# Innoptech/OpenFDCM

Hardware: AMD Instinct MI355X
Metric: template matches/sec (DT3 build + DefaultMatch/BatchOptimize search per frame) (higher is better)
Workload: dtype f32

## Files before the change

### openfdcm_amd/csrc/fdcm_capi.cpp

```cpp
#include <algorithm>
#include <cfloat>
#include <cmath>
#include <cstdlib>
#include <condition_variable>
#include <cstring>
#include <deque>
#include <functional>
#include <mutex>
#include <numeric>
#include <thread>

#include "fdcm_internal.h"
#include "fdcm_sweep.h"

namespace fdcm {
int device_cus(int device) {
    static std::mutex mu;
    static int cached[64] = {};
    std::lock_guard<std::mutex> lock(mu);
    int& c = cached[device & 63];
    if (c <= 0) FDCM_HIP(hipDeviceGetAttribute(&c, hipDeviceAttributeMultiprocessorCount, device));
    return c;
}
const char* last_error_cstr();
static thread_local int g_device = 0;

template <class F>
static int guarded(F&& f) {
    try {
        f();
        return FDCM_OK;
    } catch (const HipError& e) {
        set_error(std::string("HIP error: ") + hipGetErrorString(e.code) + " in " + e.what);
        return FDCM_EHIP;
    } catch (const std::string& s) {
        set_error(s);
        return FDCM_EINVAL;
    } catch (const std::exception& e) {
        set_error(e.what());
        return FDCM_EINTERNAL;
    } catch (...) {
        set_error("unknown error");
        return FDCM_EINTERNAL;
    }
}

static void require(bool ok, const char* msg) {
    if (!ok) throw std::string(msg);
}

template <class F>
static void records_call(fdcm_match** out, F&& call) {
    *out = nullptr;
    try {
        call();
    } catch (...) {
        result_release(*out);
        *out = nullptr;
        throw;
    }
    if (!*out) *out = result_acquire(sizeof(fdcm_match));
}

static void upload_keys_only(fdcm_featuremap* fm) {
    BuildPlan keys_only;
    keys_only.W = fm->W; keys_only.H = fm->H; keys_only.m = fm->m; keys_only.keys = fm->keys;
    const BuildLayout L = build_layout(keys_only, fm->distance, 3);
    fm->off_keys = L.off_keys;
    fm->build.plan.reserve(std::max<size_t>(16, L.plan));
    if (!fm->keys.empty())
        FDCM_HIP(hipMemcpy((char*)fm->build.plan.p + fm->off_keys, fm->keys.data(), fm->keys.size() * sizeof(float), hipMemcpyHostToDevice));
}

static void destroy(fdcm_featuremap* fm) {
    if (!fm) return;
    (void)hipSetDevice(fm->device);
    if (fm->stream) (void)hipStreamSynchronize(fm->stream);
    if (fm->prep_stream) (void)hipStreamSynchronize(fm->prep_stream);
    fm->vol.release(); fm->ivol.release(); fm->build.release(); fm->search.release();
    fm->coverage.release(); fm->coverage_stage.release();
    if (fm->timing.created)
        for (auto& e : fm->timing.ev) (void)hipEventDestroy(e);
    if (fm->stream) (void)hipStreamDestroy(fm->stream);
// ... 339 lines not shown
}

int fdcm_featuremap_from_slices(const float* keys, int64_t depth, const float* volume_host, int64_t width,
                                int64_t height, const float scene_translation[2], fdcm_featuremap** out) {
    fdcm_featuremap* fm = nullptr;
    int rc = guarded([&] {
        require(out && scene_translation, "null argument");
        require(depth >= 0 && width >= 0 && height >= 0, "negative size");
        require(depth == 0 || (keys && volume_host), "null keys/volume");
        for (int64_t i = 1; i < depth; ++i) require(keys[i - 1] < keys[i], "keys must be strictly ascending (std::map order)");
        fm = new fdcm_featuremap();
        fm->device = g_device;
        FDCM_HIP(hipSetDevice(fm->device));
        fm->depth_param = depth; fm->m = depth; fm->W = width; fm->H = height;
        fm->tx = scene_translation[0]; fm->ty = scene_translation[1];
        fm->keys.assign(keys, keys + depth);
        require(width <= 16384 && height <= 16384, "feature size above 16384 is not supported");
        const size_t sl = ivol_slice_floats(width, height);
        if (depth && sl) {
            fm->vol.reserve((size_t)depth * sl * sizeof(float));
            std::vector<float> tmp(sl, 0.f);
            for (int64_t k = 0; k < depth; ++k) {
                slice_from_xy(volume_host + (size_t)k * width * height, tmp.data(), width, height);
                FDCM_HIP(hipMemcpy(fm->vol.as<float>() + (size_t)k * sl, tmp.data(), sl * sizeof(float), hipMemcpyHostToDevice));
            }
        }
        fm->holds = VolStage::integrated;
        upload_keys_only(fm);
        *out = fm;
    });
    if (rc != FDCM_OK) { destroy(fm); if (out) *out = nullptr; }
    return rc;
}

static void check_offsets(const int64_t* off, int64_t n, const char* what) {
    require(off != nullptr, what);
    require(off[0] == 0, "offsets[0] must be 0");
    for (int64_t i = 0; i < n; ++i) require(off[i] <= off[i + 1], "offsets must be ascending");
}

int fdcm_featuremap_minmax_translation_batch(const fdcm_featuremap* fm, const float* tmpl_lines, const int64_t* line_offsets,
                                             int64_t n_templates, const float* align_vecs, float* out_minmax) {
    return guarded([&] {
        require(fm != nullptr, "featuremap is null");
        require(n_templates >= 0, "negative template count");
        if (n_templates == 0) return;
        check_offsets(line_offsets, n_templates, "line_offsets is null");
        require(line_offsets[n_templates] == 0 || tmpl_lines, "tmpl_lines is null");
        require(align_vecs && out_minmax, "null align_vecs/out_minmax");
        run_minmax(const_cast<fdcm_featuremap*>(fm), tmpl_lines, line_offsets, n_templates, align_vecs, out_minmax);
    });
}

int fdcm_featuremap_minmax_translation(const fdcm_featuremap* fm, const float* tmpl_lines, int64_t n_lines,
                                       const float align_vec[2], float out_minmax[2]) {
    const int64_t off[2] = {0, n_lines};
    if (n_lines < 0) { set_error("negative line count"); return FDCM_EINVAL; }
    return fdcm_featuremap_minmax_translation_batch(fm, tmpl_lines, off, 1, align_vec, out_minmax);
}

int fdcm_featuremap_evaluate(const fdcm_featuremap* fm, const float* tmpl_lines, const int64_t* line_offsets,
                             int64_t n_templates, const float* translations, const int64_t* translation_offsets,
                             float* scores_out) {
    return guarded([&] {
        require(fm != nullptr, "featuremap is null");
        require(n_templates >= 0, "negative template count");
        if (n_templates == 0) return;
        check_offsets(line_offsets, n_templates, "line_offsets is null");
        check_offsets(translation_offsets, n_templates, "translation_offsets is null");
        require(line_offsets[n_templates] == 0 || tmpl_lines, "tmpl_lines is null");
        require(translation_offsets[n_templates] == 0 || (translations && scores_out), "null translations/scores_out");
        run_evaluate(const_cast<fdcm_featuremap*>(fm), tmpl_lines, line_offsets, n_templates, translations, translation_offsets,
                     scores_out);
    });
}

static int create_templates(const float* lines, const int64_t* offsets, int64_t n_templates, const float* caps, fdcm_templates** out,
                            int32_t footprint = FDCM_FOOTPRINT_BOX) {
    fdcm_templates* t = nullptr;
    int rc = guarded([&] {
        require(out != nullptr, "out is null");
        require(n_templates >= 0 && (n_templates == 0 || offsets), "bad offsets");
        t = new fdcm_templates();
        t->device = g_device;
        t->footprint = footprint;
        FDCM_HIP(hipSetDevice(t->device));
        t->T = n_templates;
        t->offsets.assign(n_templates + 1, 0);
        for (int64_t i = 0; i <= n_templates && offsets; ++i) t->offsets[i] = offsets[i];
        require(t->offsets[0] == 0, "offsets[0] must be 0");
        for (int64_t i = 0; i < n_templates; ++i) require(t->offsets[i] <= t->offsets[i + 1], "offsets must be ascending");
        t->n_lines = t->offsets[n_templates];
        require(t->n_lines == 0 || lines, "lines is null");
        t->lines.assign(lines, lines + 4 * t->n_lines);
        t->lengths.resize((size_t)t->n_lines);
        t->sorted.resize((size_t)t->n_lines);
        for (int64_t i = 0; i < t->n_lines; ++i) {
            const float dx = lines[4 * i + 2] - lines[4 * i], dy = lines[4 * i + 3] - lines[4 * i + 1];
            t->lengths[i] = std::sqrt(dx * dx + dy * dy);
        }
        t->caps.assign((size_t)t->n_lines, f_inf());
        for (int64_t i = 0; i < t->n_lines && caps; ++i) {
            t->caps[i] = caps[i] == 0.f ? 0.f : caps[i];
            t->capped = t->capped || caps[i] < f_inf();
        }
        std::vector<long> ind;
        for (int64_t i = 0; i < n_templates; ++i) {
            const int64_t l0 = t->offsets[i], n = t->offsets[i + 1] - l0;
            t->max_lines = std::max(t->max_lines, n);
            ind.resize((size_t)n);
            std::iota(ind.begin(), ind.end(), 0);
            const float* len = t->lengths.data() + l0;
            std::sort(ind.begin(), ind.end(), [len](long const i1, long const i2) { return len[i1] > len[i2]; });
            for (int64_t j = 0; j < n; ++j) t->sorted[l0 + j] = (int32_t)ind[j];
        }
        t->d_lines.reserve(std::max<size_t>(16, t->lines.size() * 4));
        t->d_offsets.reserve((size_t)(n_templates + 1) * 8);
        t->d_lengths.reserve(std::max<size_t>(16, t->lengths.size() * 4));
        t->d_sorted.reserve(std::max<size_t>(16, t->sorted.size() * 4));
        if (t->n_lines) {
            FDCM_HIP(hipMemcpy(t->d_lines.p, t->lines.data(), t->lines.size() * 4, hipMemcpyHostToDevice));
            FDCM_HIP(hipMemcpy(t->d_lengths.p, t->lengths.data(), t->lengths.size() * 4, hipMemcpyHostToDevice));
            FDCM_HIP(hipMemcpy(t->d_sorted.p, t->sorted.data(), t->sorted.size() * 4, hipMemcpyHostToDevice));
        }
        FDCM_HIP(hipMemcpy(t->d_offsets.p, t->offsets.data(), (size_t)(n_templates + 1) * 8, hipMemcpyHostToDevice));
        *out = t;
    });
    if (rc != FDCM_OK) { if (t) fdcm_templates_free(t); if (out) *out = nullptr; }
    return rc;
}

int fdcm_templates_create(const float* lines, const int64_t* offsets, int64_t n_templates, fdcm_templates** out) {
    return create_templates(lines, offsets, n_templates, nullptr, out);
}

int fdcm_templates_create_capped(const float* lines, const int64_t* offsets, int64_t n_templates, const float* caps,
                                 fdcm_templates** out) {
    int rc = guarded([&] {
        require(out != nullptr, "out is null");
        require(n_templates >= 0 && (n_templates == 0 || offsets), "bad offsets");
        if (!caps || n_templates == 0) return;
        require(offsets[0] == 0, "offsets[0] must be 0");
        for (int64_t i = 0; i < n_templates; ++i) require(offsets[i] <= offsets[i + 1], "offsets must be ascending");
        for (int64_t i = 0; i < offsets[n_templates]; ++i) require(caps[i] >= 0.f, "caps must be >= 0 or +inf, never NaN");
    });
    if (rc != FDCM_OK) { if (out) *out = nullptr; return rc; }
    return create_templates(lines, offsets, n_templates, caps, out);
}

int fdcm_templates_create_shaped(const float* lines, const int64_t* offsets, int64_t n_templates, const float* caps, int32_t footprint,
                                 fdcm_templates** out) {
    int rc = guarded([&] {
        require(footprint == FDCM_FOOTPRINT_BOX || footprint == FDCM_FOOTPRINT_HULL, "footprint must be FDCM_FOOTPRINT_BOX or FDCM_FOOTPRINT_HULL");
        require(out != nullptr, "out is null");
        require(n_templates >= 0 && (n_templates == 0 || offsets), "bad offsets");
        if (!caps || n_templates == 0) return;
        require(offsets[0] == 0, "offsets[0] must be 0");
        for (int64_t i = 0; i < n_templates; ++i) require(offsets[i] <= offsets[i + 1], "offsets must be ascending");
        for (int64_t i = 0; i < offsets[n_templates]; ++i) require(caps[i] >= 0.f, "caps must be >= 0 or +inf, never NaN");
    });
    if (rc != FDCM_OK) { if (out) *out = nullptr; return rc; }
    return create_templates(lines, offsets, n_templates, caps, out, footprint);
}

int fdcm_templates_footprint_kind(const fdcm_templates* t, int32_t* kind) {
    return guarded([&] {
// ... 1235 lines not shown
```

### openfdcm_amd/csrc/fdcm_internal.h

```cpp
#pragma once
#include <hip/hip_runtime.h>
#include <stdint.h>
#include <algorithm>
#include <cstdlib>
#include <cstring>
#include <mutex>
#include <string>
#include <vector>

#include "../../include/fdcm.h"
#include "fdcm_math.h"

namespace fdcm {

void set_error(const std::string& msg);
struct HipError { hipError_t code; const char* what; int line; };
#define FDCM_HIP(call)                                                              \
    do {                                                                            \
        hipError_t e__ = (call);                                                    \
        if (e__ != hipSuccess) throw ::fdcm::HipError{e__, #call, __LINE__};        \
    } while (0)

struct TestSwitches {
    bool literal_sweep, sweep_order;
// ... 71 lines not shown
    std::vector<PropStep> prop;
    std::vector<IntegralDesc> integral;
    std::vector<LineBox> boxes;
    SeedSource seeds;
};

struct BuildLayout {
    bool empty = true;
    bool balanced = false;
    int HW64 = 0, slots = 0;
    long nchunks = 0;
    size_t vol = 0, ivol = 0, bitmap = 0, coldesc = 0, colmask = 0, offtab = 0, stack = 0;
    size_t labels = 0;
    size_t edge_parent = 0, edge_roots = 0;
    size_t pyr = 0, pyr_b = 0;
    size_t o_ent = 0, o_own = 0, o_ord = 0, o_cost = 0, o_steals = 0;
    size_t off_raster = 0, off_prop = 0, off_integral = 0, off_keys = 0, off_slice = 0, off_pixels = 0, off_cost = 0, plan = 0;
};
void make_build_plan(const float* lines, int64_t n, int64_t depth, float coeff, float padding, BuildPlan& plan);
void plan_keys(int64_t depth, std::vector<float>& keys);
void make_shape_plan(int64_t depth, float coeff, int64_t W, int64_t H, BuildPlan& plan);
void sweep_cost_proxy(const BuildPlan& plan, std::vector<int32_t>& cost);

FDCM_HD float lin_spaced_value(int mode, float low, float high, float step, int n, int i) {
    if (mode == 0) return low;
    const int size1 = (n == 1) ? 1 : n - 1;
    if (mode == 2) return (i == 0) ? low : (high - (float)(size1 - i) * step);
    return (i == size1) ? high : (low + (float)i * step);
}

static constexpr size_t kSlicePad = 1088;
FDCM_HD size_t ivol_slice_floats(int64_t W, int64_t H) { return (size_t)((W + 3) / 4) * (size_t)H * 4 + kSlicePad; }
FDCM_HD size_t ivol_index(int x, int y, int64_t H) { return ((size_t)(x >> 2) * (size_t)H + (size_t)y) * 4 + (size_t)(x & 3); }
inline void slice_to_xy(const float* il, float* xy, int64_t W, int64_t H) {
    for (int64_t x = 0; x < W; ++x)
        for (int64_t y = 0; y < H; ++y) xy[(size_t)x * H + y] = il[ivol_index((int)x, (int)y, H)];
}
inline void slice_from_xy(const float* xy, float* il, int64_t W, int64_t H) {
    for (int64_t x = 0; x < W; ++x)
        for (int64_t y = 0; y < H; ++y) il[ivol_index((int)x, (int)y, H)] = xy[(size_t)x * H + y];
}
enum class VolStage { none, transforms, propagated, integrated };

struct Timing { hipEvent_t ev[9] = {}; bool created = false; };

struct SweepHistory { long cost_chunks = 0; int cost_w = 0; size_t steals_off = 0; void reset() { *this = SweepHistory{}; } };
struct GroupTable { int m = 0, steps = 0; void reset() { *this = GroupTable{}; } };
struct BuildRecord {
    bool pending = false;
    bool seeds_fused = false;
    bool stage_events = false, total_events = false;
    float host_ms = 0.f;
    void reset() { *this = BuildRecord{}; }
};
struct BuildBuffers {
    DevBuf bitmap;
    DevBuf coldesc;
    DevBuf colmask;
    DevBuf labels;
    DevBuf edge_parent, edge_roots;
    DevBuf pyr;
    DevBuf offtab;
    DevBuf stack;
    DevBuf plan; PinnedBuf stage;
    void release() { for (DevBuf* b : {&bitmap, &coldesc, &colmask, &labels, &edge_parent, &edge_roots, &pyr, &offtab, &stack, &plan}) b->release(); stage.release(); }
};
struct SearchBuffers {
    DevBuf scene;
    DevBuf pairs;
    DevBuf records, flags;
    DevBuf out;
    DevBuf work;
    DevBuf tail, tail_out;
    DevBuf eval;
    DevBuf counter;
    DevBuf bins;
    DevBuf eval_spans;
    PinnedBuf stage, bins_stage, eval_stage;
    PinnedBuf cnt;
    void release() {
        for (DevBuf* b : {&scene, &pairs, &records, &flags, &out, &work, &tail, &tail_out, &eval, &eval_spans, &counter, &bins}) b->release();
        for (PinnedBuf* b : {&stage, &bins_stage, &eval_stage, &cnt}) b->release();
    }
};

}

struct fdcm_featuremap {
    int device = 0;
    hipStream_t stream = nullptr;
    hipStream_t prep_stream = nullptr;
    hipEvent_t prep_done = nullptr;
    int64_t depth_param = 0;
    float coeff = 0, padding = 0;
    int distance = 0;
    bool pixel_seeded = false;
    int want_stage_events = 1;
    bool shares_gpu = false;
    int64_t W = 0, H = 0, m = 0;
    float tx = 0, ty = 0;
    std::vector<float> keys;
    size_t off_keys = 0;
    fdcm::DevBuf vol;
    fdcm::DevBuf ivol;
    fdcm::VolStage holds = fdcm::VolStage::none;
    const float* current() const { return holds == fdcm::VolStage::propagated ? ivol.as<float>() : vol.as<float>(); }
    fdcm::BuildBuffers build;
    fdcm::SweepHistory sweep;
    fdcm::GroupTable groups;
    fdcm::BuildRecord built;
    int* steal_counter() const { return sweep.steals_off ? (int*)((char*)build.stack.p + sweep.steals_off) : nullptr; }
    fdcm::SearchBuffers search;
    fdcm::DevBuf coverage;
    fdcm::PinnedBuf coverage_stage;
    std::mutex seam_mutex;
    int64_t last_n_out = 0;
    fdcm::Timing timing;
    fdcm_build_timing last_build = {};
    fdcm_search_timing last_search = {};
};

struct fdcm_templates {
    int device = 0;
    int64_t T = 0, n_lines = 0, max_lines = 0;
    std::vector<float> lines;
    std::vector<int64_t> offsets;
    std::vector<float> lengths;
    std::vector<float> caps;
    bool capped = false;
    int32_t footprint = 0;
    std::vector<int32_t> sorted;
    fdcm::DevBuf d_lines, d_offsets, d_lengths, d_sorted;
};

namespace fdcm {
void ensure_stream(fdcm_featuremap* fm);
BuildLayout build_layout(const BuildPlan& plan, int distance, int stop_after);
void reserve_build(fdcm_featuremap* fm, const BuildLayout& L);
void run_build(fdcm_featuremap* fm, const BuildPlan& plan, int stop_after);
void launch_edge_labels(hipStream_t st, const uint8_t* image, int width, int height, int row_stride, const float* keys, int m,
                        const fdcm_edge_params& e, uint8_t* labels, int32_t* parent, uint32_t* roots);
void pyramid_size(int64_t width, int64_t height, int level, int64_t* w_out, int64_t* h_out);
const uint8_t* launch_pyramid(hipStream_t st, const uint8_t* image, int width, int height, int row_stride, int level, uint8_t* a, uint8_t* b,
                              uint8_t* last = nullptr);
void image_pyramid_host(int device, const uint8_t* image, int width, int height, int row_stride, bool on_device, int level, uint8_t* out,
                        bool out_on_device);
void launch_coldesc_labels(hipStream_t st, const uint8_t* labels, int width, int height, int border, void* desc, int W, int H,
                           int HW64, int m, unsigned* colmask, int* cost);
struct PixelScratch {
    DevBuf pixels, labels, keys, parent, counts, comps, out;
    ~PixelScratch();
    void take(DevBuf& b, size_t bytes, int id);
    const uint8_t* upload(const uint8_t* host_or_device, int width, int height, int& row_stride, bool on_device, const std::vector<float>* host_keys);
};
void edge_labels_host(int device, const uint8_t* image, int width, int height, int row_stride, int64_t depth, const fdcm_edge_params& e,
                      bool hysteresis, uint8_t* labels_out);
void lines_from_labels_host(int device, const uint8_t* labels, int width, int height, bool on_device, int m, const fdcm_line_params& lp,
                            float** lines, int64_t* n_lines);
void lines_from_image_host(int device, const uint8_t* image, int width, int height, int row_stride, bool on_device, int64_t depth,
                           const fdcm_edge_params& e, const fdcm_line_params& lp, float** lines, int64_t* n_lines);
void lines_last_timing(fdcm_lines_timing* out);
void finish_build(fdcm_featuremap* fm);
void sweep_order_counts(int64_t* from_history, int64_t* from_proxy);
int64_t search_capacity(const fdcm_templates* t, int64_t n_scene, int64_t maxT, int64_t maxS);
void run_search(fdcm_featuremap* fm, const fdcm_templates* t, const float* scene, int64_t n_scene, int64_t maxT,
                int64_t maxS, int optimizer, int64_t batch, int32_t base, fdcm_match* out_device, fdcm_match** out_host,
                int64_t* n_out);
void reserve_search(fdcm_featuremap* fm, const fdcm_templates* t, int64_t n_scene, int64_t maxT, int64_t maxS);
bool orientation_bins_on_host();
void reserve_eval(fdcm_featuremap* fm, size_t device_bytes, size_t stage_bytes);
void run_minmax(fdcm_featuremap* fm, const float* lines, const int64_t* offsets, int64_t T, const float* align, float* out);
void run_evaluate(fdcm_featuremap* fm, const float* lines, const int64_t* offsets, int64_t T, const float* translations,
                  const int64_t* tr_offsets, float* scores);
void exhaustive_window(fdcm_featuremap* fm, const fdcm_templates* t, int32_t sx, int32_t sy, fdcm_grid* out);
void run_score_map(fdcm_featuremap* fm, const fdcm_templates* t, const fdcm_rotations* rot, const fdcm_grid& g, float* out_host,
                   float* out_device);
void run_search_exhaustive(fdcm_featuremap* fm, const fdcm_templates* t, const fdcm_grid& g, int k, int32_t base,
                           fdcm_match** out, int64_t* n_out);
void run_search_exhaustive_peaks(fdcm_featuremap* fm, const fdcm_templates* t, const fdcm_grid& g, int k, int rx, int ry,
                                 int32_t base, fdcm_match** out, int64_t* n_out);
void exhaustive_rotations_window(fdcm_featuremap* fm, const fdcm_templates* t, const fdcm_rotations& rot, int32_t sx, int32_t sy,
                                 fdcm_grid* out);
void run_search_exhaustive_rotations(fdcm_featuremap* fm, const fdcm_templates* t, const fdcm_rotations& rot, const fdcm_grid& g,
                                     int k, int rx, int ry, int ra, int wrap, int32_t base, fdcm_match** out, int64_t* n_out);
void run_best_map(fdcm_featuremap* fm, const fdcm_templates* t, const fdcm_rotations* rot, const fdcm_grid& g, int penalty, float tau,
                  float* score_out, int32_t* pair_out);
void run_search_exhaustive_detect(fdcm_featuremap* fm, const fdcm_templates* t, const fdcm_rotations* rot, const fdcm_grid& g, int k,
                                  int rx, int ry, int penalty, float tau, int32_t base, fdcm_match** out, int64_t* n_out);
void run_search_exhaustive_detect_nms(fdcm_featuremap* fm, const fdcm_templates* t, const fdcm_rotations* rot, const fdcm_grid& g, int k,
                                      int permille, int margin, int penalty, float tau, int32_t base, fdcm_match** out,
                                      int32_t* boxes_out, int64_t* n_out);
void run_search_exhaustive_detect_all(fdcm_featuremap* fm, const fdcm_templates* t, const fdcm_rotations* rot, const fdcm_grid& g,
                                      float max_score, int max_det, int permille, int margin, int penalty, float tau, int32_t base,
                                      fdcm_match** out, int64_t* n_out, int32_t* boxes_out);
void run_search_exhaustive_detect_all_matched(fdcm_featuremap* fm, const fdcm_templates* t, const fdcm_rotations* rot, const fdcm_grid& g,
                                              float max_score, int max_det, int permille, int margin, int penalty, float tau,
                                              float min_matched, int gate, int32_t base, fdcm_match** out, int64_t* n_out,
                                              int32_t* boxes_out, float* matched_out);
void run_best_map_gated(fdcm_featuremap* fm, const fdcm_templates* t, const fdcm_rotations* rot, const fdcm_grid& g, int penalty, float tau,
                        float min_matched, float* score_out, int32_t* pair_out, float* matched_out);
void run_matched_fractions(fdcm_featuremap* fm, const fdcm_templates* t, const fdcm_rotations* rot, const int32_t* poses, int64_t n,
                           float* fractions);
void templates_matched_totals(const fdcm_templates* t, float* totals);
void detect_score_bounds(const fdcm_templates* t, int penalty, float tau, float max_score, float* bounds);
float detect_score_bound(float den, float max_score);
void templates_footprints(const fdcm_templates* t, const fdcm_rotations* rot, int margin, int32_t* boxes_out);
// ... 106 lines not shown
```

### openfdcm_amd/csrc/fdcm_search.hip

```cpp
#include <algorithm>
#include <cstdio>
#include <atomic>
#include <chrono>
#include <cstring>
#include <numeric>
#include <thread>

#include "fdcm_internal.h"
#include "fdcm_score.h"

namespace fdcm {

struct SearchParams {
    const float* vol;
    const float* keys;
    int W, H, m;
    float tx, ty;
    const float* tlines;
    const long long* toffsets;
    const float* tlengths;
    const int* tsorted;
    int T;
    const float* slines;
    const float* s_sorted_len;
// ... 337 lines not shown
        const float trx = best_k == 0 ? 0.f : (float)best_k * savx, try_ = best_k == 0 ? 0.f : (float)best_k * savy;
        r.transform[0] = T[0]; r.transform[1] = T[1]; r.transform[2] = T[2] + trx;
        r.transform[3] = T[3]; r.transform[4] = T[4]; r.transform[5] = T[5] + try_;
        if (valid) P.records[cand] = r;
        P.flags[cand] = valid ? 1 : 0;
        P.evals[cand] = (int)n_eval;
    }
}

static constexpr int kChunk = 1024;
__global__ void __launch_bounds__(256) k_chunk_counts(const int* __restrict__ flags, const int* __restrict__ evals,
                                                      long long n, int* __restrict__ counts, int* __restrict__ evsums) {
    __shared__ int part[4], epart[4];
    const long long c0 = (long long)blockIdx.x * kChunk;
    int s = 0, e = 0;
    for (int i = threadIdx.x; i < kChunk; i += 256) {
        if (c0 + i < n) { s += flags[c0 + i]; e += evals[c0 + i]; }
    }
    for (int d = 32; d >= 1; d >>= 1) { s += __shfl_xor(s, d); e += __shfl_xor(e, d); }
    if ((threadIdx.x & 63) == 0) { part[threadIdx.x >> 6] = s; epart[threadIdx.x >> 6] = e; }
    __syncthreads();
    if (threadIdx.x == 0) {
        counts[blockIdx.x] = part[0] + part[1] + part[2] + part[3];
        evsums[blockIdx.x] = epart[0] + epart[1] + epart[2] + epart[3];
    }
}
__global__ void __launch_bounds__(1024) k_scatter(const fdcm_match* __restrict__ records, const int* __restrict__ flags,
                                                  long long n, const int* __restrict__ counts,
                                                  const int* __restrict__ evsums, int nchunks,
                                                  fdcm_match* __restrict__ out, unsigned long long* __restrict__ counters,
                                                  fdcm_match* __restrict__ out2, unsigned long long* __restrict__ counters2) {
    __shared__ long long wsum[16];
    __shared__ long long chunk_base;
    const int tid = threadIdx.x, lane = tid & 63, wave = tid >> 6;
    long long s = 0;
    for (int i = tid; i < (int)blockIdx.x; i += 1024) s += counts[i];
    for (int d = 32; d >= 1; d >>= 1) s += __shfl_xor(s, d);
    if (lane == 0) wsum[wave] = s;
    __syncthreads();
    if (tid == 0) {
        long long b = 0;
        for (int w = 0; w < 16; ++w) b += wsum[w];
        chunk_base = b;
    }
    __syncthreads();
    const long long i = (long long)blockIdx.x * kChunk + tid;
    const int f = i < n ? flags[i] : 0;
    int incl = f;
    for (int d = 1; d < 64; d <<= 1) {
        const int o = __shfl_up(incl, d);
        if (lane >= d) incl += o;
    }
    __syncthreads();
    if (lane == 63) wsum[wave] = incl;
    __syncthreads();
    long long wbase = 0;
    for (int w = 0; w < wave; ++w) wbase += wsum[w];
    if (f) {
        const fdcm_match r = records[i];
        out[chunk_base + wbase + incl - 1] = r;
        if (out2) out2[chunk_base + wbase + incl - 1] = r;
    }
    if ((int)blockIdx.x == nchunks - 1) {
        if (tid == 1023) {
            counters[2] = (unsigned long long)(chunk_base + wbase + incl);
            if (counters2) counters2[2] = (unsigned long long)(chunk_base + wbase + incl);
        }
        long long ev = 0;
        for (int i2 = tid; i2 < nchunks; i2 += 1024) ev += evsums[i2];
        for (int d = 32; d >= 1; d >>= 1) ev += __shfl_xor(ev, d);
        __syncthreads();
        if (lane == 0) wsum[wave] = ev;
        __syncthreads();
        if (tid == 0) {
            long long tot = 0;
            for (int w = 0; w < 16; ++w) tot += wsum[w];
            counters[0] = (unsigned long long)tot;
            if (counters2) counters2[0] = (unsigned long long)tot;
        }
    }
}

static constexpr int kCompactChunks = 64;
__global__ void __launch_bounds__(1024) k_compact(const fdcm_match* __restrict__ records, const int* __restrict__ flags,
                                                  const int* __restrict__ evals, long long n, int nchunks,
                                                  fdcm_match* __restrict__ out, unsigned long long* __restrict__ counters,
                                                  fdcm_match* __restrict__ out2, unsigned long long* __restrict__ counters2) {
    __shared__ long long wsum[16];
    __shared__ long long chunk_base;
    const int tid = threadIdx.x, lane = tid & 63, wave = tid >> 6;
    const long long i = (long long)blockIdx.x * kChunk + tid;
    const int f = i < n ? flags[i] : 0;
    fdcm_match r{};
    if (f) r = records[i];
    long long s = 0;
    {
        const int4* f4 = reinterpret_cast<const int4*>(flags);
        const long long n4 = (long long)blockIdx.x * (kChunk / 4);
        for (long long q = tid; q < n4; q += 1024) { const int4 v = f4[q]; s += v.x + v.y + v.z + v.w; }
    }
    for (int d = 32; d >= 1; d >>= 1) s += __shfl_xor(s, d);
    if (lane == 0) wsum[wave] = s;
    __syncthreads();
    if (tid == 0) {
        long long b = 0;
        for (int w = 0; w < 16; ++w) b += wsum[w];
        chunk_base = b;
    }
    int incl = f;
    for (int d = 1; d < 64; d <<= 1) {
        const int o = __shfl_up(incl, d);
        if (lane >= d) incl += o;
    }
    __syncthreads();
    const long long cb = chunk_base;
    __syncthreads();
    if (lane == 63) wsum[wave] = incl;
    __syncthreads();
    long long wbase = 0;
    for (int w = 0; w < wave; ++w) wbase += wsum[w];
    if (f) {
        out[cb + wbase + incl - 1] = r;
        if (out2) out2[cb + wbase + incl - 1] = r;
    }
    if ((int)blockIdx.x == nchunks - 1) {
        if (tid == 1023) {
            counters[2] = (unsigned long long)(cb + wbase + incl);
            if (counters2) counters2[2] = (unsigned long long)(cb + wbase + incl);
        }
        long long ev = 0;
        for (long long i2 = tid; i2 < n; i2 += 1024) ev += evals[i2];
        for (int d = 32; d >= 1; d >>= 1) ev += __shfl_xor(ev, d);
        __syncthreads();
        if (lane == 0) wsum[wave] = ev;
        __syncthreads();
        if (tid == 0) {
            long long tot = 0;
            for (int w = 0; w < 16; ++w) tot += wsum[w];
            counters[0] = (unsigned long long)tot;
            if (counters2) counters2[0] = (unsigned long long)tot;
        }
    }
}

struct SearchLayout {
    int64_t maxT = 0, maxS = 0;
    std::vector<long long> coff;
    int64_t cpt_max = 0, ncand = 0, pairs_stride = 0;
    int nchunks = 0;
    size_t o_lines = 0, o_len = 0, o_idx = 0, o_coff = 0, scene = 0;
    size_t records = 0, flags = 0, counters = 64, pairs = 0, work_list = 0, work = 0, bins = 0, out = 0;
};
static SearchLayout search_layout(const fdcm_templates* t, int64_t n_scene, int64_t maxT, int64_t maxS) {
    SearchLayout L;
    L.maxT = std::min<int64_t>(std::max<int64_t>(maxT, 0), std::max<int64_t>(t->max_lines, 0));
    L.maxS = std::min<int64_t>(std::max<int64_t>(maxS, 0), n_scene);
    L.coff.assign((size_t)t->T + 1, 0);
    for (int64_t i = 0; i < t->T; ++i) {
        const int64_t nt = t->offsets[i + 1] - t->offsets[i];
        const int64_t c = 2 * std::min<int64_t>(nt, L.maxT) * L.maxS;
        L.coff[i + 1] = L.coff[i] + c;
        L.cpt_max = std::max(L.cpt_max, c);
    }
    L.ncand = L.coff[t->T];
    L.nchunks = (int)((L.ncand + kChunk - 1) / kChunk);
    L.pairs_stride = L.maxT * L.maxS;
    auto align16 = [](size_t v) { return (v + 15) & ~(size_t)15; };
    const size_t n_s = (size_t)n_scene, ncand = (size_t)L.ncand;
    L.o_len = align16(n_s * 16), L.o_idx = L.o_len + align16(n_s * 4), L.o_coff = L.o_idx + align16(n_s * 4);
    L.scene = L.o_coff + align16(L.coff.size() * 8);
    L.records = ncand * sizeof(fdcm_match);
    L.flags = 2 * (ncand + (size_t)L.nchunks) * sizeof(int);
    L.pairs = std::max<size_t>(16, (size_t)t->T * (size_t)L.pairs_stride * sizeof(int2));
    L.work_list = align16(ncand / 2 * sizeof(int2));
    L.work = L.work_list + 2 * (size_t)kWorkBins * sizeof(int);
    L.bins = ncand * (size_t)std::max<int64_t>(1, t->max_lines) * sizeof(unsigned short);
    L.out = (ncand + 1) * sizeof(fdcm_match);
    return L;
}

int64_t search_capacity(const fdcm_templates* t, int64_t n_scene, int64_t maxT, int64_t maxS) {
    return search_layout(t, n_scene, maxT, maxS).ncand;
}

bool orientation_bins_on_host() {
    static const bool on_host = [] {
        const bool forced = test_switches().host_bins;
        const bool differs = fdcm_selftest_atanf(0, 65537, (1ull << 32) / 65537) != 0;
        if (forced || differs)
            fprintf(stderr, "libfdcm_hip: orientation bins of the candidates come from this machine's libm on host threads (%s); "
                            "searches are slower than with the device's atanf (fdcm_orientation_bins_mode() == 1)\n",
                    differs ? "its atanf differs from the glibc 2.35 restatement the device runs" : "FDCM_FORCE_HOST_BINS is set");
        return forced || differs;
    }();
    return on_host;
}

static void reserve_workspaces(fdcm_featuremap* fm, const SearchLayout& L, bool host_bins) {
    fm->search.stage.reserve(L.scene); fm->search.scene.reserve(L.scene);
    fm->search.records.reserve(L.records); fm->search.flags.reserve(L.flags); fm->search.counter.reserve(L.counters);
    fm->search.pairs.reserve(L.pairs); fm->search.work.reserve(L.work);
    if (host_bins) { fm->search.bins_stage.reserve(L.bins); fm->search.bins.reserve(L.bins); }
}

void reserve_search(fdcm_featuremap* fm, const fdcm_templates* t, int64_t n_scene, int64_t maxT, int64_t maxS) {
    if (!t || t->T == 0 || n_scene <= 0) return;
    FDCM_HIP(hipSetDevice(fm->device));
    const SearchLayout L = search_layout(t, n_scene, maxT, maxS);
    if (L.ncand == 0) return;
    reserve_workspaces(fm, L, orientation_bins_on_host());
    fm->search.cnt.reserve(L.counters);
}

void run_search(fdcm_featuremap* fm, const fdcm_templates* t, const float* scene, int64_t n_scene, int64_t maxT,
                int64_t maxS, int optimizer, int64_t batch, int32_t base, fdcm_match* out_device, fdcm_match** out_host,
                int64_t* n_out) {
    *n_out = 0;
    fm->last_search = fdcm_search_timing{};
    if (t->T == 0 || n_scene == 0 || (fm->W == 0 && fm->H == 0)) return;
    const bool host_bins_needed = orientation_bins_on_host();
    FDCM_HIP(hipSetDevice(fm->device));
    ensure_stream(fm);
    hipStream_t st = fm->stream;
    const int n_s = (int)n_scene;
    const SearchLayout L = search_layout(t, n_scene, maxT, maxS);
    maxT = L.maxT; maxS = L.maxS;
    const int window = (int)maxS;
    std::vector<float> slen((size_t)n_s);
    for (int i = 0; i < n_s; ++i) {
        const float dx = scene[4 * i + 2] - scene[4 * i], dy = scene[4 * i + 3] - scene[4 * i + 1];
        slen[i] = std::sqrt(dx * dx + dy * dy);
    }
    std::vector<long> sidx((size_t)n_s);
    std::iota(sidx.begin(), sidx.end(), 0);
    std::sort(sidx.begin(), sidx.end(), [&slen](long const i1, long const i2) { return slen[i1] > slen[i2]; });
    const std::vector<long long>& coff = L.coff;
    const long long ncand = L.ncand;
    fm->last_search.candidates = ncand;
    if (ncand == 0) return;
    if (fm->holds != VolStage::integrated) throw std::string("the feature map holds a partial build (no line integral): nothing to search");
    const int64_t B = optimizer == FDCM_BATCH_OPTIMIZE ? std::max<int64_t>(1, batch) : 1;
    if (B > 4096) throw std::string("batch_size above 4096 is not supported");
    const int win = B <= 15 ? (int)((15 / B) * B) : (int)B;
    const int lds_lines = (int)std::max<int64_t>(1, t->max_lines);
    const size_t lds = (size_t)kWavesPerBlock * ((size_t)fm->m + 5 * (size_t)lds_lines + 2 * (size_t)win + 1) * sizeof(float);
    if (lds > 160 * 1024) throw std::string("scene/template too large for the search kernel's LDS staging");
    if (host_bins_needed && fm->m > 65535) throw std::string("host-side orientation bins need depth <= 65535");
    reserve_workspaces(fm, L, host_bins_needed);
    hipStream_t sp = st;
    if (!fm->shares_gpu) {
        if (!fm->prep_stream) {
            FDCM_HIP(hipStreamCreateWithFlags(&fm->prep_stream, hipStreamNonBlocking));
            FDCM_HIP(hipEventCreateWithFlags(&fm->prep_done, hipEventDisableTiming));
        }
        sp = fm->prep_stream;
    }
    if (test_switches().poison) {
        SearchBuffers& s = fm->search;
        if (!out_device) s.out.reserve(L.out);
        if (!out_host) s.cnt.reserve(L.counters);
        FDCM_HIP(hipStreamSynchronize(sp));
        poison_fill(s.scene, sp, FDCM_FILL_SCENE); poison_fill(s.pairs, sp, FDCM_FILL_PAIRS); poison_fill(s.work, sp, FDCM_FILL_WORK);
        poison_fill(s.records, st, FDCM_FILL_RECORDS); poison_fill(s.flags, st, FDCM_FILL_FLAGS); poison_fill(s.counter, st, FDCM_FILL_COUNTER);
        poison_fill(s.bins, st, FDCM_FILL_BINS);
        if (!out_device) poison_fill(s.out, st, FDCM_FILL_OUT);
        poison_fill(s.stage, FDCM_FILL_SEARCH_STAGE); poison_fill(s.bins_stage, FDCM_FILL_BINS_STAGE); poison_fill(s.cnt, FDCM_FILL_CNT);
    }
    char* hs = (char*)fm->search.stage.p;
    std::memcpy(hs + L.o_lines, scene, (size_t)n_s * 16);
    float* hl = (float*)(hs + L.o_len);
    int* hi = (int*)(hs + L.o_idx);
    for (int i = 0; i < n_s; ++i) { hl[i] = slen[sidx[i]]; hi[i] = (int)sidx[i]; }
    std::memcpy(hs + L.o_coff, coff.data(), coff.size() * 8);
    FDCM_HIP(hipMemcpyAsync(fm->search.scene.p, hs, L.scene, hipMemcpyHostToDevice, sp));
    const int nchunks = L.nchunks;
    SearchParams P{};
    P.vol = fm->vol.as<float>();
    P.keys = (const float*)((const char*)fm->build.plan.p + fm->off_keys);
    P.W = (int)fm->W; P.H = (int)fm->H; P.m = (int)fm->m; P.tx = fm->tx; P.ty = fm->ty;
    P.tlines = t->d_lines.as<float>();
    P.toffsets = t->d_offsets.as<long long>();
    P.tlengths = t->d_lengths.as<float>();
    P.tsorted = t->d_sorted.as<int>();
    P.T = (int)t->T;
    const char* ds = (const char*)fm->search.scene.p;
    P.slines = (const float*)(ds + L.o_lines);
    P.s_sorted_len = (const float*)(ds + L.o_len);
    P.s_sorted_idx = (const int*)(ds + L.o_idx);
    P.n_s = n_s;
    P.maxT = (int)maxT; P.maxS = (int)maxS; P.window = window;
    P.optimizer = optimizer;
    P.batch = (int)B;
    P.win = win;
    P.base = base;
    P.cand_offsets = (const long long*)(ds + L.o_coff);
    P.bpt = (int)((L.cpt_max + kWavesPerBlock - 1) / kWavesPerBlock);
    P.ncand = ncand;
    P.lds_lines = lds_lines;
    P.records = fm->search.records.as<fdcm_match>();
    P.flags = fm->search.flags.as<int>();
    P.evals = P.flags + ncand + nchunks;
    P.counters = fm->search.counter.as<unsigned long long>();
    P.pairs_stride = (int)L.pairs_stride;
    P.pairs = fm->search.pairs.as<int2>();
    const bool buf32 = !test_switches().search_flat && (size_t)fm->m * ivol_slice_floats(fm->W, fm->H) * sizeof(float) < ((size_t)1 << 32);
    if (lds > 64 * 1024)
        FDCM_HIP(hipFuncSetAttribute(buf32 ? (const void*)k_search<true> : (const void*)k_search<false>,
                                     hipFuncAttributeMaxDynamicSharedMemorySize, (int)lds));
    hipEvent_t* ev = fm->timing.ev;
    const bool timed = fm->want_stage_events != 0;
    if (timed) FDCM_HIP(hipEventRecord(ev[6], st));
    hipLaunchKernelGGL(k_pairs, dim3((unsigned)(((size_t)t->T * maxT + 255) / 256)), dim3(256), 0, sp, P);
    const long long n_slots = (long long)t->T * P.pairs_stride;
    if (n_slots <= 0x7fffffffll) {
        if (n_slots <= kWlSlotsPerBlock) {
            hipLaunchKernelGGL(k_worklist, dim3(1), dim3(1024), 0, sp, P, n_slots, fm->search.work.as<int2>());
        } else {
            int* ghist = (int*)((char*)fm->search.work.p + L.work_list);
            int* cursor = ghist + kWorkBins;
            const unsigned nb = (unsigned)((n_slots + kWlSlotsPerBlock - 1) / kWlSlotsPerBlock);
            FDCM_HIP(hipMemsetAsync(ghist, 0, (size_t)kWorkBins * sizeof(int), sp));
            hipLaunchKernelGGL(k_wl_count, dim3(nb), dim3(1024), 0, sp, P, n_slots, ghist);
            hipLaunchKernelGGL(k_wl_starts, dim3(1), dim3(1024), 0, sp, ghist, cursor);
            hipLaunchKernelGGL(k_wl_scatter, dim3(nb), dim3(1024), 0, sp, P, n_slots, ghist, cursor, fm->search.work.as<int2>());
        }
        P.work = fm->search.work.as<int2>();
        P.nblocks = (int)(((ncand + kWavesPerBlock - 1) / kWavesPerBlock + 7) / 8 * 8);
    } else {
        P.work = nullptr;
        P.nblocks = (int)((size_t)t->T * P.bpt);
    }
    if (sp != st) {
        FDCM_HIP(hipEventRecord(fm->prep_done, sp));
        FDCM_HIP(hipStreamWaitEvent(st, fm->prep_done, 0));
    }
    if (host_bins_needed) {
        const size_t stride = (size_t)P.lds_lines;
        unsigned short* hb = (unsigned short*)fm->search.bins_stage.p;
        const float* keys = fm->keys.data();
        const int mkeys = (int)fm->m;
        std::vector<float> sorted_len((size_t)n_s);
        for (int i = 0; i < n_s; ++i) sorted_len[i] = slen[sidx[i]];
        const unsigned nthreads = std::max(1u, std::min(16u, std::thread::hardware_concurrency()));
        std::vector<std::thread> th;
        std::atomic<int64_t> next{0};
        const fdcm_templates* tt = t;
        for (unsigned w = 0; w < nthreads; ++w)
            th.emplace_back([&, tt] {
                for (int64_t ti; (ti = next.fetch_add(1)) < tt->T;) {
                    const int64_t l0 = tt->offsets[ti];
                    const int n_t = (int)(tt->offsets[ti + 1] - l0);
                    const int jmax = (int)std::min<int64_t>(n_t, maxT);
                    for (int j = 0; j < jmax; ++j) {
                        const int tl_local = tt->sorted[(size_t)l0 + j];
                        const float tlen = tt->lengths[(size_t)l0 + tl_local];
                        const int centre = binary_search_greater(sorted_len.data(), n_s, tlen);
                        int rb, re;
                        centered_range(centre, n_s, (int)maxS, rb, re);
                        for (int wi = 0; wi < window; ++wi) {
                            const int scene_idx = (int)sidx[rb + wi];
                            float T1[6], T2[6];
                            align_pair(&tt->lines[(size_t)(l0 + tl_local) * 4], scene + (size_t)scene_idx * 4, T1, T2);
                            for (int flip = 0; flip < 2; ++flip) {
                                const float* T = flip ? T2 : T1;
                                const long long cand = coff[ti] + 2ll * (j * window + wi) + flip;
                                unsigned short* out = hb + (size_t)cand * stride;
                                for (int i = 0; i < n_t; ++i) {
                                    const float* p = &tt->lines[(size_t)(l0 + i) * 4];
                                    const float x1 = (T[0] * p[0] + T[1] * p[1]) + T[2], y1 = (T[3] * p[0] + T[4] * p[1]) + T[5];
                                    const float x2 = (T[0] * p[2] + T[1] * p[3]) + T[2], y2 = (T[3] * p[2] + T[4] * p[3]) + T[5];
                                    const float angle = std::atan((y2 - y1) / (x2 - x1));
                                    out[i] = (unsigned short)closest_orientation(keys, mkeys, angle);
                                }
                            }
                        }
                    }
                }
            });
        for (auto& x : th) x.join();
        FDCM_HIP(hipMemcpyAsync(fm->search.bins.p, hb, (size_t)ncand * stride * sizeof(unsigned short), hipMemcpyHostToDevice, st));
        P.host_bins = fm->search.bins.as<unsigned short>();
    }
    if (buf32) hipLaunchKernelGGL(k_search<true>, dim3((unsigned)P.nblocks), dim3(64 * kWavesPerBlock), lds, st, P);
    else hipLaunchKernelGGL(k_search<false>, dim3((unsigned)P.nblocks), dim3(64 * kWavesPerBlock), lds, st, P);
    fdcm_match* dst = out_device;
    if (!dst) {
        fm->search.out.reserve(L.out);
        dst = fm->search.out.as<fdcm_match>();
        P.counters = reinterpret_cast<unsigned long long*>(dst + ncand);
    }
    int* d_counts = P.flags + ncand;
    int* d_evsums = P.evals + ncand;
    fdcm_match* host_out = nullptr;
    unsigned long long* host_cnt = nullptr;
    if (out_host) {
        *out_host = result_acquire((size_t)(ncand + 1) * sizeof(fdcm_match));
        FDCM_HIP(hipHostGetDevicePointer((void**)&host_out, *out_host, 0));
        host_cnt = reinterpret_cast<unsigned long long*>(host_out + ncand);
    } else {
        fm->search.cnt.reserve(L.counters);
        FDCM_HIP(hipHostGetDevicePointer((void**)&host_cnt, fm->search.cnt.p, 0));
    }
    if (nchunks <= kCompactChunks && !test_switches().search_compact2) {
        hipLaunchKernelGGL(k_compact, dim3((unsigned)nchunks), dim3(1024), 0, st, P.records, P.flags, P.evals, ncand, nchunks, dst, P.counters,
                           host_out, host_cnt);
    } else {
        hipLaunchKernelGGL(k_chunk_counts, dim3((unsigned)nchunks), dim3(256), 0, st, P.flags, P.evals, ncand, d_counts, d_evsums);
        hipLaunchKernelGGL(k_scatter, dim3((unsigned)nchunks), dim3(1024), 0, st, P.records, P.flags, ncand, d_counts, d_evsums,
                           nchunks, dst, P.counters, host_out, host_cnt);
    }
    if (timed) FDCM_HIP(hipEventRecord(ev[7], st));
    FDCM_HIP(hipGetLastError());
    unsigned long long hc[3] = {0, 0, 0};
    FDCM_HIP(hipStreamSynchronize(st));
    finish_build(fm);
    std::memcpy(hc, out_host ? (const void*)(*out_host + ncand) : (const void*)fm->search.cnt.p, sizeof hc);
    *n_out = (int64_t)hc[2];
    fm->last_search.evaluations = (int64_t)hc[0];
    if (timed) FDCM_HIP(hipEventElapsedTime(&fm->last_search.kernel_ms, ev[6], ev[7]));
    fm->last_search.total_ms = fm->last_search.kernel_ms;
}

}
```

Before: 63.02 million.

## Cache per-template coefficient upload and coarsen compact kernel to four flags per thread

The coefficient block of the scene staging buffer is now uploaded only when the template set, sizes, or buffer identity change, tracked by a new per-template id and a key on the feature map. Other scene data is still copied every call. Separately, the single-block compaction kernel now uses 256 threads that each handle four flags loaded as an int4, with unrolled prefix-sum loops, to cut thread count and make loads wider. The cache depends on the coefficient data being a pure function of the key, and the compaction rewrite changes the output write pattern.

```diff
diff --git a/openfdcm_amd/csrc/fdcm_capi.cpp b/openfdcm_amd/csrc/fdcm_capi.cpp
--- a/openfdcm_amd/csrc/fdcm_capi.cpp
+++ b/openfdcm_amd/csrc/fdcm_capi.cpp
@@ -1,4 +1,5 @@
 #include <algorithm>
+#include <atomic>
 #include <cfloat>
 #include <cmath>
 #include <cstdlib>
@@ -504,6 +505,8 @@
         require(out != nullptr, "out is null");
         require(n_templates >= 0 && (n_templates == 0 || offsets), "bad offsets");
         t = new fdcm_templates();
+        static std::atomic<uint64_t> next_id{1};
+        t->id = next_id.fetch_add(1);
         t->device = g_device;
         t->footprint = footprint;
         FDCM_HIP(hipSetDevice(t->device));
diff --git a/openfdcm_amd/csrc/fdcm_internal.h b/openfdcm_amd/csrc/fdcm_internal.h
--- a/openfdcm_amd/csrc/fdcm_internal.h
+++ b/openfdcm_amd/csrc/fdcm_internal.h
@@ -177,6 +177,14 @@
         for (DevBuf* b : {&scene, &pairs, &records, &flags, &out, &work, &tail, &tail_out, &eval, &eval_spans, &counter, &bins}) b->release();
         for (PinnedBuf* b : {&stage, &bins_stage, &eval_stage, &cnt}) b->release();
     }
+};
+
+struct CoffKey {
+    uint64_t tset = 0;
+    int64_t maxT = -1, maxS = -1, n_s = -1;
+    const void* p = nullptr;
+    size_t cap = 0;
+    bool operator==(const CoffKey& o) const { return tset == o.tset && maxT == o.maxT && maxS == o.maxS && n_s == o.n_s && p == o.p && cap == o.cap; }
 };
 
 }
@@ -206,6 +214,7 @@
     fdcm::BuildRecord built;
     int* steal_counter() const { return sweep.steals_off ? (int*)((char*)build.stack.p + sweep.steals_off) : nullptr; }
     fdcm::SearchBuffers search;
+    fdcm::CoffKey coff_key;
     fdcm::DevBuf coverage;
     fdcm::PinnedBuf coverage_stage;
     std::mutex seam_mutex;
@@ -217,6 +226,7 @@
 
 struct fdcm_templates {
     int device = 0;
+    uint64_t id = 0;
     int64_t T = 0, n_lines = 0, max_lines = 0;
     std::vector<float> lines;
     std::vector<int64_t> offsets;
diff --git a/openfdcm_amd/csrc/fdcm_search.hip b/openfdcm_amd/csrc/fdcm_search.hip
--- a/openfdcm_amd/csrc/fdcm_search.hip
+++ b/openfdcm_amd/csrc/fdcm_search.hip
@@ -443,32 +443,50 @@
 }
 
 static constexpr int kCompactChunks = 64;
-__global__ void __launch_bounds__(1024) k_compact(const fdcm_match* __restrict__ records, const int* __restrict__ flags,
-                                                  const int* __restrict__ evals, long long n, int nchunks,
-                                                  fdcm_match* __restrict__ out, unsigned long long* __restrict__ counters,
-                                                  fdcm_match* __restrict__ out2, unsigned long long* __restrict__ counters2) {
-    __shared__ long long wsum[16];
+static constexpr int kCompactThreads = 256, kCompactPer = kChunk / kCompactThreads;
+__global__ void __launch_bounds__(kCompactThreads) k_compact(const fdcm_match* __restrict__ records, const int* __restrict__ flags,
+                                                             const int* __restrict__ evals, long long n, int nchunks,
+                                                             fdcm_match* __restrict__ out, unsigned long long* __restrict__ counters,
+                                                             fdcm_match* __restrict__ out2, unsigned long long* __restrict__ counters2) {
+    constexpr int NW = kCompactThreads / 64;
+    static_assert(kCompactPer == 4, "a thread loads its flags as one int4");
+    __shared__ long long wsum[NW];
     __shared__ long long chunk_base;
     const int tid = threadIdx.x, lane = tid & 63, wave = tid >> 6;
-    const long long i = (long long)blockIdx.x * kChunk + tid;
-    const int f = i < n ? flags[i] : 0;
-    fdcm_match r{};
-    if (f) r = records[i];
+    const long long i0 = (long long)blockIdx.x * kChunk + (long long)tid * kCompactPer;
+    int f[kCompactPer];
+    if (i0 + kCompactPer <= n) {
+        const int4 v = *reinterpret_cast<const int4*>(flags + i0);
+        f[0] = v.x; f[1] = v.y; f[2] = v.z; f[3] = v.w;
+    } else {
+#pragma unroll
+        for (int q = 0; q < kCompactPer; ++q) f[q] = i0 + q < n ? flags[i0 + q] : 0;
+    }
+    constexpr int RW = sizeof(fdcm_match) / sizeof(int);
+    int r[kCompactPer][RW];
+#pragma unroll
+    for (int q = 0; q < kCompactPer; ++q) {
+        const int* src = reinterpret_cast<const int*>(records + i0 + q);
+#pragma unroll
+        for (int c = 0; c < RW; ++c) r[q][c] = f[q] ? src[c] : 0;
+    }
     long long s = 0;
     {
         const int4* f4 = reinterpret_cast<const int4*>(flags);
         const long long n4 = (long long)blockIdx.x * (kChunk / 4);
-        for (long long q = tid; q < n4; q += 1024) { const int4 v = f4[q]; s += v.x + v.y + v.z + v.w; }
+#pragma unroll 4
+        for (long long q = tid; q < n4; q += kCompactThreads) { const int4 v = f4[q]; s += v.x + v.y + v.z + v.w; }
     }
     for (int d = 32; d >= 1; d >>= 1) s += __shfl_xor(s, d);
     if (lane == 0) wsum[wave] = s;
     __syncthreads();
     if (tid == 0) {
         long long b = 0;
-        for (int w = 0; w < 16; ++w) b += wsum[w];
+        for (int w = 0; w < NW; ++w) b += wsum[w];
         chunk_base = b;
     }
-    int incl = f;
+    const int mine = f[0] + f[1] + f[2] + f[3];
+    int incl = mine;
     for (int d = 1; d < 64; d <<= 1) {
         const int o = __shfl_up(incl, d);
         if (lane >= d) incl += o;
@@ -480,24 +498,34 @@
     __syncthreads();
     long long wbase = 0;
     for (int w = 0; w < wave; ++w) wbase += wsum[w];
-    if (f) {
-        out[cb + wbase + incl - 1] = r;
-        if (out2) out2[cb + wbase + incl - 1] = r;
+    long long pos = cb + wbase + incl - mine;
+#pragma unroll
+    for (int q = 0; q < kCompactPer; ++q) {
+        if (!f[q]) continue;
+        int* d1 = reinterpret_cast<int*>(out + pos);
+        int* d2 = reinterpret_cast<int*>(out2 + pos);
+#pragma unroll
+        for (int c = 0; c < RW; ++c) {
+            d1[c] = r[q][c];
+            if (out2) d2[c] = r[q][c];
+        }
+        ++pos;
     }
     if ((int)blockIdx.x == nchunks - 1) {
-        if (tid == 1023) {
+        if (tid == kCompactThreads - 1) {
             counters[2] = (unsigned long long)(cb + wbase + incl);
             if (counters2) counters2[2] = (unsigned long long)(cb + wbase + incl);
         }
         long long ev = 0;
-        for (long long i2 = tid; i2 < n; i2 += 1024) ev += evals[i2];
+#pragma unroll 8
+        for (long long i2 = tid; i2 < n; i2 += kCompactThreads) ev += evals[i2];
         for (int d = 32; d >= 1; d >>= 1) ev += __shfl_xor(ev, d);
         __syncthreads();
         if (lane == 0) wsum[wave] = ev;
         __syncthreads();
         if (tid == 0) {
             long long tot = 0;
-            for (int w = 0; w < 16; ++w) tot += wsum[w];
+            for (int w = 0; w < NW; ++w) tot += wsum[w];
             counters[0] = (unsigned long long)tot;
             if (counters2) counters2[0] = (unsigned long long)tot;
         }
@@ -626,14 +654,21 @@
         poison_fill(s.bins, st, FDCM_FILL_BINS);
         if (!out_device) poison_fill(s.out, st, FDCM_FILL_OUT);
         poison_fill(s.stage, FDCM_FILL_SEARCH_STAGE); poison_fill(s.bins_stage, FDCM_FILL_BINS_STAGE); poison_fill(s.cnt, FDCM_FILL_CNT);
+        fm->coff_key = CoffKey{};
     }
     char* hs = (char*)fm->search.stage.p;
     std::memcpy(hs + L.o_lines, scene, (size_t)n_s * 16);
     float* hl = (float*)(hs + L.o_len);
     int* hi = (int*)(hs + L.o_idx);
     for (int i = 0; i < n_s; ++i) { hl[i] = slen[sidx[i]]; hi[i] = (int)sidx[i]; }
-    std::memcpy(hs + L.o_coff, coff.data(), coff.size() * 8);
-    FDCM_HIP(hipMemcpyAsync(fm->search.scene.p, hs, L.scene, hipMemcpyHostToDevice, sp));
+    FDCM_HIP(hipMemcpyAsync(fm->search.scene.p, hs, L.o_coff, hipMemcpyHostToDevice, sp));
+    const CoffKey key{t->id, L.maxT, L.maxS, n_s, fm->search.scene.p, fm->search.scene.cap};
+    if (!(key == fm->coff_key)) {
+        fm->coff_key = CoffKey{};
+        std::memcpy(hs + L.o_coff, coff.data(), coff.size() * 8);
+        FDCM_HIP(hipMemcpyAsync((char*)fm->search.scene.p + L.o_coff, hs + L.o_coff, coff.size() * 8, hipMemcpyHostToDevice, sp));
+        fm->coff_key = key;
+    }
     const int nchunks = L.nchunks;
     SearchParams P{};
     P.vol = fm->vol.as<float>();
@@ -763,7 +798,7 @@
         FDCM_HIP(hipHostGetDevicePointer((void**)&host_cnt, fm->search.cnt.p, 0));
     }
     if (nchunks <= kCompactChunks && !test_switches().search_compact2) {
-        hipLaunchKernelGGL(k_compact, dim3((unsigned)nchunks), dim3(1024), 0, st, P.records, P.flags, P.evals, ncand, nchunks, dst, P.counters,
+        hipLaunchKernelGGL(k_compact, dim3((unsigned)nchunks), dim3(kCompactThreads), 0, st, P.records, P.flags, P.evals, ncand, nchunks, dst, P.counters,
                            host_out, host_cnt);
     } else {
         hipLaunchKernelGGL(k_chunk_counts, dim3((unsigned)nchunks), dim3(256), 0, st, P.flags, P.evals, ncand, d_counts, d_evsums);
```

After: 62.29 million. 0.988x the previous value.
